# Amos-Chen98/neo-planner

Measured on AMD Instinct MI355X. Metric: trajectories/sec (batched replan), higher is better.
Workload: dtype f32x; 1 GPU; cfg2: 40 x 4096 trajectories x 20 waypoints per step per GPU, 1 x 300^3 f32 ESDF per GPU (trilinear, pillars + 80 canopy boxes), each optimised to L-BFGS-B termination; batch_per_launch=4096, pieces=21, dims=3, esdf_voxels=27000000, layout=brick, parallelism=scene-sharded x1, launches_in_flight_per_gpu=4

## Files before the change

### neo-planner_amd/csrc/neo_group_kernel.hpp

```cpp
#pragma once
#include "neo_device.hpp"
#include "neo_lbfgs_sm.hpp"

namespace neo {

template <int D, int W, int NS, typename Real, class MapT, class LookupT, int SU, typename Num = double>
struct GroupBackend {
  using Hist = Num;
  struct Vec {
    Num v[NS];
  };
  Traj<D, D, Num> t;
  const DevParams &prm;
  const MapT &map;
  double *xs;
  double *sc;
  LineSearch *lsp;
  double *cst;
  Hist *hist;
  int m;

  __device__ GroupBackend(const DevParams &p, const MapT &mp) : prm(p), map(mp) {}

  __device__ __forceinline__ double dot(const Vec &a, const Vec &b) const {
    Num s = Num(0);
#pragma unroll
    for (int k = 0; k < NS; ++k) s += a.v[k] * b.v[k];
    return GroupLanes<W>::sum(s);
  }
  __device__ __forceinline__ double amax(const Vec &a) const {
    Num s = Num(0);
#pragma unroll
    for (int k = 0; k < NS; ++k) s = fmax(s, fabs(a.v[k]));
    return GroupLanes<W>::max_nonneg(s);
  }
  __device__ __forceinline__ void copy(Vec &d, const Vec &s) const {
#pragma unroll
    for (int k = 0; k < NS; ++k) d.v[k] = s.v[k];
  }
  __device__ __forceinline__ void neg(Vec &d, const Vec &s) const {
#pragma unroll
    for (int k = 0; k < NS; ++k) d.v[k] = -s.v[k];
  }
  __device__ __forceinline__ void axpy(double a, const Vec &x, Vec &y) const {
#pragma unroll
    for (int k = 0; k < NS; ++k) y.v[k] += (Num)a * x.v[k];
  }
  __device__ __forceinline__ void lincomb(Vec &o, const Vec &a, double s, const Vec &b) const {
#pragma unroll
    for (int k = 0; k < NS; ++k) o.v[k] = a.v[k] + (Num)s * b.v[k];
  }
  __device__ __forceinline__ void scale(Vec &v, double s) const {
#pragma unroll
    for (int k = 0; k < NS; ++k) v.v[k] *= (Num)s;
  }
  __device__ __forceinline__ void hist_put(int slot, const Vec &s, const Vec &y) {
    const int gl = GroupLanes<W>::lane();
#pragma unroll
    for (int k = 0; k < NS; ++k)
      if (k * W + gl < t.n) {
        hist[slot * t.n + k * W + gl] = s.v[k];
        hist[(m + slot) * t.n + k * W + gl] = y.v[k];
      }
    lds_wave_sync();
  }
  __device__ __forceinline__ void hist_get(int row, Vec &v) const {
    const int gl = GroupLanes<W>::lane();
#pragma unroll
    for (int k = 0; k < NS; ++k) v.v[k] = (k * W + gl < t.n) ? hist[row * t.n + k * W + gl] : Num(0);
  }
  __device__ __forceinline__ void hist_get_s(int slot, Vec &v) const { hist_get(slot, v); }
  __device__ __forceinline__ void hist_get_y(int slot, Vec &v) const { hist_get(m + slot, v); }
  __device__ __forceinline__ void hist_get_sy(int slot, Vec &s, Vec &y) const {
    hist_get(slot, s);
    hist_get(m + slot, y);
  }
  __device__ __forceinline__ void sput(int i, double v) {
    sc[i] = v;
    lds_wave_sync();
  }
  __device__ __forceinline__ double sget(int i) const { return sc[i]; }
  __device__ __forceinline__ double sdiff(int i, double b) const { return sget(i) - b; }
  __device__ __forceinline__ double rho_dot(int slot, const Vec &a, const Vec &b) const { return sget(slot) * dot(a, b); }
  __device__ __forceinline__ double uni(double v) const { return v; }
  __device__ __forceinline__ LineSearch &ls() { return *lsp; }
  __device__ __forceinline__ double *cost_store() { return cst; }
  __device__ __forceinline__ void note_eval(int, int, double, double, const Vec &, const Vec &) {}

  __device__ __forceinline__ int eval(const Vec &x, double &f, Vec &g, double (&costs)[4], int &nsamp) {
    const int lane = GroupLanes<W>::lane();
    const int M = t.M;
    Num *xn = reinterpret_cast<Num *>(xs);
    lds_wave_sync();
#pragma unroll
    for (int k = 0; k < NS; ++k)
      if (k * W + lane < t.n) xn[k * W + lane] = x.v[k];
    lds_wave_sync();
    const bool act = lane < M;
    t.tau = act ? xn[t.nq + lane] : Num(0);
#pragma unroll
    for (int d = 0; d < D; ++d) {
      t.P0[d] = (lane == 0 || !act) ? bstate<D, GroupLanes<W>, false>(t, 0, d) : xn[d * (M - 1) + (lane > 0 ? lane - 1 : 0)];
      t.P1[d] = (lane >= M - 1) ? bstate<D, GroupLanes<W>, true>(t, 0, d) : xn[d * (M - 1) + lane];
    }
    double energy = 0.0, tsum = 0.0;
    const int st = minco_forward<D, GroupLanes<W>, Num>(t, prm, energy, tsum);
    nsamp = GroupLanes<W>::sum(act ? t.ns : 0);
    Num gC[6][D], gT = Num(0);
    double cf, ck;
    {
      Real cr[6][D], gCr[6][D], gTr;
#pragma unroll
      for (int k = 0; k < 6; ++k)
#pragma unroll
        for (int d = 0; d < D; ++d) cr[k][d] = (Real)t.c[k][d];
      LookupT lk(map);
      const SampleLanes sl = group_sample_lanes<GroupLanes<W>>(M, t.ns);
      minco_sample<Real, D, LookupT, SU, false, GroupLanes<W>>(M, sl, t.ns, cr, prm, lk, gCr, gTr, cf, ck);
#pragma unroll
      for (int k = 0; k < 6; ++k)
#pragma unroll
        for (int d = 0; d < D; ++d) gC[k][d] = (Num)gCr[k][d];
      gT = (Num)gTr;
    }
    costs[0] = energy;
    costs[1] = tsum;
    costs[2] = cf;
    costs[3] = ck;
    f = costs[0] * prm.w[0] + costs[1] * prm.w[1] + costs[2] * prm.w[2] + costs[3] * prm.w[3];
    Num gq[D], gtau;
    const int bst = minco_backward<D, GroupLanes<W>, Num>(t, prm, gC, gT, gq, gtau);
    lds_wave_sync();
    if (lane >= 1 && lane < M) {
#pragma unroll
      for (int d = 0; d < D; ++d) xn[d * (M - 1) + lane - 1] = gq[d];
    }
    if (lane < M) xn[t.nq + lane] = gtau;
    lds_wave_sync();
#pragma unroll
    for (int k = 0; k < NS; ++k) g.v[k] = (k * W + lane < t.n) ? xn[k * W + lane] : Num(0);
    if (st != 0) {
      f = 0.0;
#pragma unroll
      for (int k = 0; k < 4; ++k) costs[k] = 0.0;
      return st;
    }
    return bst;
  }
};

#ifndef NEO_GRP_OCC
#define NEO_GRP_OCC 1
#endif
#ifndef NEO_GRP_OCC_F32
#define NEO_GRP_OCC_F32 2
#endif
#ifndef NEO_GRP_U
#define NEO_GRP_U 2
#endif
template <int D, typename Real, class MapT, class LookupT, int W, int NS, typename Num = double>
__global__ __launch_bounds__(kWave, (sizeof(Num) == 4 ? NEO_GRP_OCC_F32 : NEO_GRP_OCC)) void optimize_group_kernel(int B, int M, DevParams prm, const MapT *maps,
                                                                   const double *x0, double *x,
                                                                   const double *__restrict__ head,
                                                                   const double *__restrict__ tail,
                                                                   double *__restrict__ costs4,
                                                                   double *__restrict__ costs4_last,
                                                                   int *__restrict__ nit, int *__restrict__ nfev,
                                                                   int *__restrict__ status,
                                                                   long long *__restrict__ nsamples,
                                                                   const int *__restrict__ order,
                                                                   int *__restrict__ ticket) {
  constexpr int G = kWave / W;
  __shared__ double xs[G][W * NS];
  __shared__ double sc[G][2 * NEO_LBFGS_M];
  __shared__ LineSearch lsm[G];
  __shared__ double cst[G][12];
  __shared__ Num bnd[G][6 * D];
  extern __shared__ double dyn_lds[];
  using BE = GroupBackend<D, W, NS, Real, MapT, LookupT, NEO_GRP_U, Num>;
  const MapT map = maps[0];
  BE be(prm, map);
  be.t = Traj<D, D, Num>{};
  const int gl = GroupLanes<W>::lane();
  const int g = lane_id() / W;
  const int nq = D * (M - 1), n = nq + M;
  be.xs = xs[g];
  be.sc = sc[g];
  be.lsp = &lsm[g];
  be.cst = cst[g];
  be.m = NEO_LBFGS_M;
  be.hist = reinterpret_cast<typename BE::Hist *>(dyn_lds) + (size_t)g * 2 * NEO_LBFGS_M * n;
  be.t.M = M;
  be.t.nq = nq;
  be.t.n = n;
  be.t.L = GroupLanes<W>::lanes_per_piece(M);
  be.t.bnd = bnd[g];

  LbfgsOpts o{prm.ftol, prm.gtol, prm.maxls, prm.maxiter, prm.maxfun, NEO_LBFGS_M};
  LbfgsMachine<BE> mach(be, o);
  int b = 0;
  bool busy = false;
  long long samples = 0;

  auto take = [&]() {
    int tk = 0;
    if (gl == 0) tk = atomicAdd(ticket, 1);
    tk = __shfl(tk, GroupLanes<W>::base(), kWave);
    busy = tk < B;
    b = busy ? (order ? order[tk] : tk) : 0;
    be.t.head = head + (size_t)b * 3 * D;
    be.t.tail = tail + (size_t)b * 3 * D;
    lds_wave_sync();
    for (int e = gl; e < 6 * D; e += W)
      bnd[g][e] = (Num)(e < 3 * D ? be.t.head[e] : be.t.tail[e - 3 * D]);
    lds_wave_sync();
#pragma unroll
    for (int k = 0; k < NS; ++k) mach.x.v[k] = (k * W + gl < n) ? x0[(size_t)b * n + k * W + gl] : 0.0;
    mach.begin();
    samples = 0;
  };
  auto put = [&]() {
#pragma unroll
    for (int k = 0; k < NS; ++k)
      if (k * W + gl < n) x[(size_t)b * n + k * W + gl] = mach.x.v[k];
    if (gl == 0) {
      LbfgsResult res;
      mach.result(res);
      int st = res.status;
      if (res.costs_last[3] * prm.w[3] > prm.coll_tol) st |= NEO_TRAJ_FLAG_COLLISION;
#pragma unroll
      for (int k = 0; k < 4; ++k) {
        costs4[(size_t)b * 4 + k] = res.costs[k];
        if (costs4_last) costs4_last[(size_t)b * 4 + k] = res.costs_last[k];
      }
      nit[b] = res.nit;
      nfev[b] = res.nfev;
      status[b] = st;
      if (nsamples) nsamples[b] = samples;
    }
  };

  take();
  while (__any(busy)) {
    double fnew, c4[4];
    typename BE::Vec gnew;
    int ns;
    const int est = be.eval(mach.x, fnew, gnew, c4, ns);
    if (busy) {
      mach.f = fnew;
      mach.g = gnew;
#pragma unroll
      for (int k = 0; k < 4; ++k) be.cst[k] = c4[k];
      samples += ns;
      mach.advance(est);
      if (!mach.need_eval()) {
        put();
        take();
      }
    }
  }
}

}
```

### neo-planner_amd/csrc/neo_kernels.hpp

```cpp
#pragma once
#include <type_traits>
#include <hip/hip_runtime.h>
#include <hip/hip_fp16.h>

#include "../../include/neo_planner.h"
#ifndef NEO_FUSED_U
#define NEO_FUSED_U (sizeof(Real) == 4 ? 4 : 2)
#endif
#ifndef NEO_W2_U
#define NEO_W2_U 1
#endif
#ifndef NEO_W2_OCC
#define NEO_W2_OCC 2
#endif
#ifndef NEO_X_OCC
#define NEO_X_OCC 3
#endif
#ifndef NEO_SM_MAX_SLOTS
#define NEO_SM_MAX_SLOTS 2
#endif
#ifndef NEO_W2_MAX_SLOTS
#define NEO_W2_MAX_SLOTS 4
#endif
#include "neo_device.hpp"
#include "neo_lbfgs.hpp"
#include "neo_lbfgs_sm.hpp"

namespace neo {

template <typename Num, int NS>
using opt_scalar_t = std::conditional_t<sizeof(Num) == 4 && (NS <= NEO_SM_MAX_SLOTS), float, double>;

template <int D, int NS, typename Real>
__host__ __device__ constexpr int stage_doubles() {
  constexpr int fold = sizeof(Real) == 4 ? kWave * 8 * D * (int)sizeof(Real) : 0;
  return (NS * kWave * 8 > fold ? NS * kWave * 8 : fold) / 8;
}

constexpr int kSlCacheInts = kWave / 4 + kWave + 4;

template <typename Real, int NS, int WAVES>
__host__ __device__ constexpr bool pairs_in_f32() {
  return sizeof(Real) == 4 && WAVES == 2 && NS > 2;
}
template <int D, int NS, typename Real, class MapT, class LookupT, int SU = NEO_FUSED_U, class LG = WaveLanes,
          bool PAIRS32 = false, typename Num = double, class Plan = PlanDynamic>
struct DevBackend {
  static constexpr int DL = LG::dl(D);
  static constexpr int kSlotsN = NS;
  static constexpr bool kPcr = sizeof(Num) == 4 && LG::W == kWave;
  static constexpr bool kAhead = !Plan::dynamic && Plan::gather_ahead && LookupT::gather_ahead && SU == 1 && sizeof(Real) == 4;
  struct Vec {
    Num v[NS];
  };
  Traj<D, DL, Num> t;
  const DevParams &prm;
  const MapT &map;
  double *xs;
  static constexpr int kStage = stage_doubles<D, NS, Real>();
  int *sl_cache = nullptr;
  bool fold_rows = true;
  bool fold_acc = false;
  using Scalar = opt_scalar_t<Num, NS>;
  LineSearchT<Scalar> *lsp;
  double *cst;
  using Hist = std::conditional_t<PAIRS32, float, double>;
  Hist *hist;
  int npad, m;
  double *coeff_out;
  long long samples = 0;
  int last_ns = 0;
  double *trace = nullptr;
  double *trace_xg = nullptr;
  int trace_cap = 0;

  __device__ DevBackend(const DevParams &p, const MapT &mp) : prm(p), map(mp) {}

  __device__ __forceinline__ double dot(const Vec &a, const Vec &b) const {
    Num s = Num(0);
#pragma unroll
    for (int k = 0; k < NS; ++k) s += a.v[k] * b.v[k];
    return uni((double)wave_sum(s));
  }
  __device__ __forceinline__ double uni(double v) const { return uniform(v); }
  __device__ __forceinline__ float uni(float v) const { return uniform(v); }
  __device__ __forceinline__ double amax(const Vec &a) const {
    Num s = Num(0);
#pragma unroll
    for (int k = 0; k < NS; ++k) s = fmax(s, fabs(a.v[k]));
    return wave_max_nonneg(s);
  }
  __device__ __forceinline__ void copy(Vec &d, const Vec &s) const {
#pragma unroll
    for (int k = 0; k < NS; ++k) d.v[k] = s.v[k];
  }
  __device__ __forceinline__ void neg(Vec &d, const Vec &s) const {
#pragma unroll
    for (int k = 0; k < NS; ++k) d.v[k] = -s.v[k];
  }
  __device__ __forceinline__ void axpy(double a, const Vec &x, Vec &y) const {
#pragma unroll
    for (int k = 0; k < NS; ++k) y.v[k] += (Num)a * x.v[k];
  }
  __device__ __forceinline__ void lincomb(Vec &o, const Vec &a, double s, const Vec &b) const {
#pragma unroll
    for (int k = 0; k < NS; ++k) o.v[k] = a.v[k] + (Num)s * b.v[k];
  }
  __device__ __forceinline__ void scale(Vec &v, double s) const {
#pragma unroll
    for (int k = 0; k < NS; ++k) v.v[k] *= (Num)s;
  }
  static constexpr int kFull = NS == 3 ? 2 : NS / 2;
  __device__ __forceinline__ bool in_range(int k, int lane) const { return k < kFull || k * kWave + lane < t.n; }
  __device__ __forceinline__ void hist_put(int slot, const Vec &s, const Vec &y) {
    const int lane = lane_id();
#pragma unroll
    for (int k = 0; k < NS; ++k)
      if (in_range(k, lane)) {
        hist[slot * t.n + k * kWave + lane] = (Hist)s.v[k];
        hist[(m + slot) * t.n + k * kWave + lane] = (Hist)y.v[k];
      }
    lds_wave_sync();
  }
  __device__ __forceinline__ void hist_get(int row, Vec &v) const {
    const int lane = lane_id();
#pragma unroll
    for (int k = 0; k < NS; ++k) v.v[k] = in_range(k, lane) ? (Num)hist[row * t.n + k * kWave + lane] : Num(0);
  }
  __device__ __forceinline__ void hist_get_s(int slot, Vec &v) const { hist_get(slot, v); }
  __device__ __forceinline__ void hist_get_y(int slot, Vec &v) const { hist_get(m + slot, v); }
  __device__ __forceinline__ void hist_get_sy(int slot, Vec &s, Vec &y) const {
    const int lane = lane_id();
    const Hist *ps = hist + slot * t.n + lane, *py = hist + (m + slot) * t.n + lane;
#pragma unroll
    for (int k = 0; k < NS; ++k) {
      s.v[k] = Num(0);
      y.v[k] = Num(0);
      if (in_range(k, lane)) {
        s.v[k] = (Num)ps[k * kWave];
        y.v[k] = (Num)py[k * kWave];
      }
    }
  }
  Num sreg = Num(0);
  __device__ __forceinline__ void sput(int i, double v) { sreg = (lane_id() == i) ? (Num)v : sreg; }
  __device__ __forceinline__ double sget(int i) const { return (double)rdlane(sreg, i); }
  __device__ __forceinline__ double sdiff(int i, double b) const { return (double)(rdlane(sreg, i) - (Num)b); }
  __device__ __forceinline__ double rho_dot(int slot, const Vec &a, const Vec &b) const {
    Num s = Num(0);
#pragma unroll
    for (int k = 0; k < NS; ++k) s += a.v[k] * b.v[k];
    return (double)(rdlane(sreg, slot) * wave_sum(s));
  }
  static constexpr bool kOwnDirection = sizeof(Num) == 4;
  __device__ __forceinline__ void dot3(const Vec &a0, const Vec &b0, const Vec &a1, const Vec &b1, const Vec &a2, const Vec &b2,
                                       Num &t0, Num &t1, Num &t2) const {
    Num p0 = Num(0), p1 = Num(0), p2 = Num(0);
#pragma unroll
    for (int k = 0; k < NS; ++k) {
      p0 += a0.v[k] * b0.v[k];
      p1 += a1.v[k] * b1.v[k];
      p2 += a2.v[k] * b2.v[k];
    }
    Num unused;
    wave_sum4((float)p0, (float)p1, (float)p2, 0.0f, t0, t1, t2, unused);
  }
  __device__ __forceinline__ void direction(const Vec &g, Vec &d, int col, int head, int mm, Num theta) {
    if (col == 0) {
      neg(d, g);
      return;
    }
    if constexpr (!Plan::dynamic && Plan::hist_ahead) {
      if (col == NEO_LBFGS_M) {
        direction_full(g, d, head, mm, theta);
        return;
      }
    }
    auto slot_of = [&](int k) { return head + k < mm ? head + k : head + k - mm; };
    copy(d, g);
    Vec sA, yA, sB, yB;
    int k = col - 1;
    for (; k >= 1; k -= 2) {
      const int A = slot_of(k), B = slot_of(k - 1);
      hist_get_sy(A, sA, yA);
      hist_get_sy(B, sB, yB);
      Num t0, t1, t2;
      dot3(sA, d, sB, d, sB, yA, t0, t1, t2);
      const Num aA = rdlane(sreg, A) * t0;
      const Num aB = rdlane(sreg, B) * (t1 - aA * t2);
      sput(mm + A, (double)aA);
      sput(mm + B, (double)aB);
#pragma unroll
      for (int q = 0; q < NS; ++q) d.v[q] = (d.v[q] - aA * yA.v[q]) - aB * yB.v[q];
    }
    if (k == 0) {
      const int A = slot_of(0);
      hist_get_sy(A, sA, yA);
      const Num aA = (Num)rho_dot(A, sA, d);
      sput(mm + A, (double)aA);
      axpy(-(double)aA, yA, d);
    }
    scale(d, (double)(Num(1) / theta));
    k = 0;
    for (; k + 1 < col; k += 2) {
      const int A = slot_of(k), B = slot_of(k + 1);
      hist_get_sy(A, sA, yA);
      hist_get_sy(B, sB, yB);
      Num t0, t1, t2;
      dot3(yA, d, yB, d, yB, sA, t0, t1, t2);
      const Num cA = rdlane(sreg, mm + A) - rdlane(sreg, A) * t0;
      const Num cB = rdlane(sreg, mm + B) - rdlane(sreg, B) * (t1 + cA * t2);
#pragma unroll
      for (int q = 0; q < NS; ++q) d.v[q] = (d.v[q] + cA * sA.v[q]) + cB * sB.v[q];
    }
    if (k < col) {
      const int A = slot_of(k);
      hist_get_sy(A, sA, yA);
      const double b = rho_dot(A, yA, d);
      axpy(sdiff(mm + A, b), sA, d);
    }
    scale(d, -1.0);
  }
  template <int COL>
  struct DirFull {
    DevBackend &be;
    Vec &d;
    const Num inv_theta;
    int off[NS];
    Vec s[COL], y[COL];
    Num alpha[COL];
    __device__ __forceinline__ void settle(Vec &sv, Vec &yv) const {
#pragma unroll
      for (int k = kFull; k < NS; ++k)
        if (lane_ge(be.t.n - k * kWave)) {
          sv.v[k] = Num(0);
          yv.v[k] = Num(0);
        }
    }
    template <int K>
    __device__ __forceinline__ void read(int slot) {
      const Hist *ps = be.hist + slot * be.t.n, *py = be.hist + (be.m + slot) * be.t.n;
#pragma unroll
      for (int k = 0; k < NS; ++k) {
        s[K].v[k] = (Num)ps[off[k]];
        y[K].v[k] = (Num)py[off[k]];
      }
    }
    template <int KA, int KB>
    __device__ __forceinline__ void pair1(int A, int B) {
      settle(s[KA], y[KA]);
      settle(s[KB], y[KB]);
      Num t0, t1, t2;
      be.dot3(s[KA], d, s[KB], d, s[KB], y[KA], t0, t1, t2);
      const Num aA = rdlane(be.sreg, A) * t0;
      const Num aB = rdlane(be.sreg, B) * (t1 - aA * t2);
      alpha[KA] = aA;
      alpha[KB] = aB;
#pragma unroll
      for (int q = 0; q < NS; ++q) d.v[q] = (d.v[q] - aA * y[KA].v[q]) - aB * y[KB].v[q];
    }
    template <int KA, int KB>
    __device__ __forceinline__ void pair2(int A, int B) {
      Num t0, t1, t2;
      be.dot3(y[KA], d, y[KB], d, y[KB], s[KA], t0, t1, t2);
      const Num cA = alpha[KA] - rdlane(be.sreg, A) * t0;
      const Num cB = alpha[KB] - rdlane(be.sreg, B) * (t1 + cA * t2);
#pragma unroll
      for (int q = 0; q < NS; ++q) d.v[q] = (d.v[q] + cA * s[KA].v[q]) + cB * s[KB].v[q];
    }
    template <int K>
    __device__ __forceinline__ void single1(int A) {
      settle(s[K], y[K]);
      const Num aA = (Num)be.rho_dot(A, s[K], d);
      alpha[K] = aA;
      be.axpy(-(double)aA, y[K], d);
    }
    template <int K>
    __device__ __forceinline__ void single2(int A) {
      const double b = be.rho_dot(A, y[K], d);
      be.axpy((double)(alpha[K] - (Num)b), s[K], d);
    }
    __device__ __forceinline__ void seam() { be.scale(d, (double)inv_theta); }
  };
  __device__ __forceinline__ void direction_full(const Vec &g, Vec &d, int head, int mm, Num theta) {
    copy(d, g);
    DirFull<NEO_LBFGS_M> w{*this, d, Num(1) / theta};
    const int lane = lane_id();
#pragma unroll
    for (int k = 0; k < NS; ++k) w.off[k] = in_range(k, lane) ? k * kWave + lane : 0;
    hist_walk_full<NEO_LBFGS_M>(head, mm, w);
    scale(d, -1.0);
  }

  __device__ __forceinline__ LineSearchT<Scalar> &ls() { return *lsp; }
  __device__ __forceinline__ double *cost_store() { return cst; }

  __device__ __forceinline__ void note_eval(int nfev, int iter, double stp, double f, const Vec &x, const Vec &g) {
    if constexpr (!Plan::dynamic && !Plan::trace) return;
    if (nfev > trace_cap) return;
    if (trace != nullptr && lane_id() == 0) {
      double *r = trace + (size_t)(nfev - 1) * 4;
      r[0] = f;
      r[1] = stp;
      r[2] = (double)last_ns;
      r[3] = (double)iter;
    }
    if (trace_xg != nullptr) {
      const int lane = lane_id();
      double *r = trace_xg + (size_t)(nfev - 1) * 2 * t.n;
#pragma unroll
      for (int k = 0; k < NS; ++k)
        if (k * kWave + lane < t.n) {
          r[k * kWave + lane] = (double)x.v[k];
          r[t.n + k * kWave + lane] = (double)g.v[k];
        }
    }
  }

  __device__ __forceinline__ void scatter_x(const Vec &x) {
    const int lane = opaque(lane_id());
    lds_wave_sync();
    Num *xn = reinterpret_cast<Num *>(xs);
#pragma unroll
    for (int k = 0; k < NS; ++k)
      if (in_range(k, lane)) xn[k * kWave + lane] = x.v[k];
    lds_wave_sync();
    const int M = t.M;
    const int p = opaque(LG::piece());
    const bool act = p < M;
    t.tau = act ? xn[t.nq + p] : Num(0);
#pragma unroll
    for (int d = 0; d < DL; ++d) {
      const int dg = LG::dim0() + d;
      t.P0[d] = (p == 0 || !act) ? bstate<D, LG, false>(t, 0, d) : xn[dg * (M - 1) + (p > 0 ? p - 1 : 0)];
      t.P1[d] = (p >= M - 1) ? bstate<D, LG, true>(t, 0, d) : xn[dg * (M - 1) + p];
    }
  }

  __device__ __forceinline__ int eval(const Vec &x, double &f, Vec &g, double *costs) {
    const int lane = lane_id();
    const int p = LG::piece();
    NEO_MARK("eval_begin");
    const int M_all = t.M;
    t.M = opaque_uniform(M_all);
    scatter_x(x);
    NEO_MARK("scatter_done");
    Num *xn = reinterpret_cast<Num *>(xs);
    double energy, tsum;
    const int st = minco_forward<D, LG, Num, kPcr, Plan>(t, prm, energy, tsum);
    NEO_MARK("forward_done");
    if (st != 0) {
      f = 0.0;
#pragma unroll
      for (int k = 0; k < 4; ++k) costs[k] = 0.0;
      return st;
    }
    if (plan_pick<Plan, Plan::coeff_out>(coeff_out != nullptr) && p < t.M) {
#pragma unroll
      for (int k = 0; k < 6; ++k)
#pragma unroll
        for (int d = 0; d < DL; ++d) coeff_out[(size_t)(6 * p + k) * D + LG::dim0() + d] = (double)t.c[k][d];
    }
    Num gC[6][DL], gT = Num(0);
    double cf, ck;
    {
      Real cr[6][DL], gCr[6][DL], gTr;
#pragma unroll
      for (int k = 0; k < 6; ++k)
#pragma unroll
        for (int d = 0; d < DL; ++d) cr[k][d] = (Real)t.c[k][d];
      LookupT lk(map);
      int ns_by_piece = t.ns;
      if constexpr (LG::S > 1) ns_by_piece = __shfl(t.ns, min(LG::S * lane, kWave - 1), kWave);
      NEO_MARK("assign_begin");
      t.M = opaque_uniform(M_all);
      SampleLanes sl;
      bool cached = false;
      const int ns_key = lane < t.M ? ns_by_piece : 0;
      const bool have_cache = plan_pick<Plan, Plan::sl_cache>(sl_cache != nullptr);
      if (have_cache) cached = __ballot(ns_key == (int)reinterpret_cast<const unsigned char *>(sl_cache)[lane]) == ~0ull;
      if (cached) {
        const unsigned pk = (unsigned)sl_cache[kWave / 4 + lane];
        sl.piece = pk & 63;
        sl.r = (pk >> 6) & 63;
        sl.L = (pk >> 12) & 127;
        sl.act = ((pk >> 19) & 1) != 0;
        sl.first = (pk >> 20) & 63;
        sl.Lp = pk >> 26;
        sl.rounds = __builtin_amdgcn_readfirstlane(sl_cache[kWave / 4 + kWave]);
        sl.lmax = __builtin_amdgcn_readfirstlane(sl_cache[kWave / 4 + kWave + 1]);
        sl.total = __builtin_amdgcn_readfirstlane(sl_cache[kWave / 4 + kWave + 2]);
      } else {
        sl = balanced_sample_lanes<kAhead>(t.M, ns_by_piece, reinterpret_cast<int *>(xs));
        if (have_cache) {
          const bool fits = sl.lmax < 64 && ns_key < 255;
          reinterpret_cast<unsigned char *>(sl_cache)[lane] = (unsigned char)(__ballot(!fits) == 0 ? ns_key : 255);
          sl_cache[kWave / 4 + lane] = (int)((unsigned)sl.piece | ((unsigned)sl.r << 6) | ((unsigned)sl.L << 12) |
                                             ((sl.act ? 1u : 0u) << 19) | ((unsigned)sl.first << 20) | ((unsigned)sl.Lp << 26));
          if (lane == 0) {
            sl_cache[kWave / 4 + kWave] = sl.rounds;
            sl_cache[kWave / 4 + kWave + 1] = sl.lmax;
            sl_cache[kWave / 4 + kWave + 2] = sl.total;
          }
          lds_wave_sync();
        }
      }
      last_ns = sl.total;
      samples += (long long)last_ns;
      NEO_MARK("assign_done");
      minco_sample<Real, D, LookupT, SU, false, LG, Plan>(
          t.M, sl, t.ns, cr, prm, lk, gCr, gTr, cf, ck,
          plan_pick<Plan, Plan::fold_rows>(fold_rows) ? reinterpret_cast<Real *>(xs) : nullptr, fold_acc);
#pragma unroll
      for (int k = 0; k < 6; ++k)
#pragma unroll
        for (int d = 0; d < DL; ++d) gC[k][d] = (Num)gCr[k][d];
      gT = (Num)gTr;
    }
    costs[0] = uniform(energy);
    costs[1] = uniform(tsum);
    costs[2] = uniform(cf);
    costs[3] = uniform(ck);
    f = uniform(costs[0] * prm.w[0] + costs[1] * prm.w[1] + costs[2] * prm.w[2] + costs[3] * prm.w[3]);
    Num gq[DL], gtau;
    NEO_MARK("sample_done");
    t.M = opaque_uniform(M_all);
    if constexpr (kAhead && sizeof(Num) == 4) {
      const Num i1 = opaque(t.i1);
      t.i2 = i1 * i1;
      t.i3 = t.i2 * i1;
      t.i4 = t.i2 * t.i2;
    }
    const int bst = minco_backward<D, LG, Num, kPcr, Plan>(t, prm, gC, gT, gq, gtau);
    NEO_MARK("backward_done");
    if (bst != 0) return bst;
    lds_wave_sync();
    const int pg = opaque(p), lg = opaque(lane);
    if (pg >= 1 && pg < t.M) {
#pragma unroll
      for (int d = 0; d < DL; ++d) xn[(LG::dim0() + d) * (t.M - 1) + pg - 1] = gq[d];
    }
    if (pg < t.M && LG::dim0() == opaque_uniform(0)) xn[t.nq + pg] = gtau;
    lds_wave_sync();
#pragma unroll
    for (int k = 0; k < NS; ++k) g.v[k] = in_range(k, lg) ? xn[k * kWave + lg] : Num(0);
    NEO_MARK("gather_done");
    return 0;
  }
};

__host__ __device__ inline size_t opt_state_doubles(int n, int m) { return 64 + 5 * (size_t)n + kWave + 2 * (size_t)m * (size_t)n; }

template <class BE, class Mach>
__device__ __forceinline__ void save_run(BE &be, const Mach &mc, double *st) {
  const int lane = lane_id(), n = be.t.n;
  lds_wave_sync();
  if (lane == 0) {
    const int iv[9] = {mc.phase, mc.status, mc.nfev, mc.nit, mc.iter, mc.col, mc.head, mc.task, mc.ifun};
#pragma unroll
    for (int k = 0; k < 9; ++k) st[k] = (double)iv[k];
    const double dv[7] = {(double)mc.f, (double)mc.fold, (double)mc.stp, (double)mc.gd, (double)mc.gdold, (double)mc.theta,
                          (double)mc.stp_evaluated};
#pragma unroll
    for (int k = 0; k < 7; ++k) st[9 + k] = dv[k];
    st[16] = (double)be.samples;
    st[17] = (double)be.last_ns;
    const auto &L = *be.lsp;
    const double lv[20] = {(double)L.ftol, (double)L.gtol, (double)L.xtol, (double)L.stpmin, (double)L.stpmax, (double)L.brackt,
                           (double)L.stage, (double)L.ginit, (double)L.gtest, (double)L.gx, (double)L.gy, (double)L.finit,
                           (double)L.fx, (double)L.fy, (double)L.stx, (double)L.sty, (double)L.stmin, (double)L.stmax,
                           (double)L.width, (double)L.width1};
#pragma unroll
    for (int k = 0; k < 20; ++k) st[20 + k] = lv[k];
#pragma unroll
    for (int k = 0; k < 12; ++k) st[40 + k] = be.cst[k];
  }
  double *v = st + 64;
#pragma unroll
  for (int k = 0; k < BE::kSlotsN; ++k)
    if (k * kWave + lane < n) {
      const int e = k * kWave + lane;
      v[e] = (double)mc.x.v[k];
      v[n + e] = (double)mc.g.v[k];
      v[2 * n + e] = (double)mc.t.v[k];
      v[3 * n + e] = (double)mc.r.v[k];
      v[4 * n + e] = (double)mc.d.v[k];
    }
  v[5 * n + lane] = (double)be.sreg;
  double *h = v + 5 * n + kWave;
  for (int i = lane; i < 2 * be.m * n; i += kWave) h[i] = (double)be.hist[i];
}

template <class BE, class Mach>
__device__ __forceinline__ void load_run(BE &be, Mach &mc, const double *st) {
  using Num = decltype(be.sreg);
  const int lane = lane_id(), n = be.t.n;
  auto iu = [&](int k) { return (int)uniform(st[k]); };
  mc.phase = iu(0); mc.status = iu(1); mc.nfev = iu(2); mc.nit = iu(3); mc.iter = iu(4);
  mc.col = iu(5); mc.head = iu(6); mc.task = iu(7); mc.ifun = iu(8);
  using S = typename Mach::S;
  mc.f = (S)uniform(st[9]); mc.fold = (S)uniform(st[10]); mc.stp = (S)uniform(st[11]); mc.gd = (S)uniform(st[12]);
  mc.gdold = (S)uniform(st[13]); mc.theta = (S)uniform(st[14]); mc.stp_evaluated = (S)uniform(st[15]);
  be.samples = (long long)uniform(st[16]);
  be.last_ns = iu(17);
  if (lane == 0) {
    auto &L = *be.lsp;
    L.ftol = (S)st[20]; L.gtol = (S)st[21]; L.xtol = (S)st[22]; L.stpmin = (S)st[23]; L.stpmax = (S)st[24];
    L.brackt = (int)st[25]; L.stage = (int)st[26];
    L.ginit = (S)st[27]; L.gtest = (S)st[28]; L.gx = (S)st[29]; L.gy = (S)st[30]; L.finit = (S)st[31]; L.fx = (S)st[32];
    L.fy = (S)st[33]; L.stx = (S)st[34]; L.sty = (S)st[35]; L.stmin = (S)st[36]; L.stmax = (S)st[37]; L.width = (S)st[38];
    L.width1 = (S)st[39];
#pragma unroll
    for (int k = 0; k < 12; ++k) be.cst[k] = st[40 + k];
  }
  const double *v = st + 64;
#pragma unroll
  for (int k = 0; k < BE::kSlotsN; ++k) {
    const int e = k * kWave + lane;
    const bool in = e < n;
    mc.x.v[k] = in ? (Num)v[e] : Num(0);
    mc.g.v[k] = in ? (Num)v[n + e] : Num(0);
    mc.t.v[k] = in ? (Num)v[2 * n + e] : Num(0);
    mc.r.v[k] = in ? (Num)v[3 * n + e] : Num(0);
    mc.d.v[k] = in ? (Num)v[4 * n + e] : Num(0);
  }
  be.sreg = (Num)v[5 * n + lane];
  const double *h = v + 5 * n + kWave;
  for (int i = lane; i < 2 * be.m * n; i += kWave) be.hist[i] = (typename BE::Hist)h[i];
  lds_wave_sync();
}

template <class LG = WaveLanes, int D, int DL, typename Num>
__device__ __forceinline__ void load_boundary(Traj<D, DL, Num> &t, const double *head, const double *tail, int M,
                                              Num *bnd_lds = nullptr) {
  t.M = M;
  t.nq = D * (M - 1);
  t.n = t.nq + M;
  t.L = sample_lanes_per_piece(M);
  t.head = head;
  t.tail = tail;
  stage_boundary<D, LG>(t, bnd_lds);
}

struct MapTable {
  const void *maps;
};

template <int D, int NS, typename Real, class MapT, class LookupT, class LG = WaveLanes, typename Num = double>
__global__ __launch_bounds__(kWave) void eval_kernel(int B, int M, DevParams prm, MapT map,
                                                      const double *__restrict__ x,
                                                      const double *__restrict__ head,
                                                      const double *__restrict__ tail,
                                                      double *__restrict__ cost, double *__restrict__ costs4,
                                                      double *__restrict__ grad, double *__restrict__ coeffs,
                                                      int *__restrict__ status) {
  __shared__ __attribute__((aligned(16))) double xs[stage_doubles<D, NS, Real>()];
  __shared__ LineSearchT<opt_scalar_t<Num, NS>> lsm;
  __shared__ double cst[12];
  __shared__ Num bnd[6 * D];
  constexpr bool kKeep = sizeof(Num) == 4 && LG::S > 1;
  __shared__ __attribute__((aligned(16))) Num mult_s[kKeep ? (5 * 8 + 4) * (kWave / LG::S + 1) : 4];
  const int b = blockIdx.x;
  if (b >= B) return;
  using BE = DevBackend<D, NS, Real, MapT, LookupT, NEO_FUSED_U, LG, false, Num>;
  BE be(prm, map);
  if constexpr (kKeep) be.t.pcr_mult = mult_s;
  be.xs = xs;
  if constexpr (sizeof(Num) == 4 && LG::W == kWave)
    if (pcr_xch_elems(M, LG::dl(D)) * (int)sizeof(Num) <= stage_doubles<D, NS, Real>() * 8) be.t.pcr_xch = reinterpret_cast<Num *>(xs);
  be.lsp = &lsm;
  be.cst = cst;
  be.hist = nullptr;
  be.m = NEO_LBFGS_M;
  load_boundary<LG>(be.t, head + (size_t)b * 3 * D, tail + (size_t)b * 3 * D, M, bnd);
  const int n = be.t.n;
  be.npad = NS * kWave;
  be.coeff_out = coeffs ? coeffs + (size_t)b * 6 * M * D : nullptr;
  const int lane = lane_id();
  typename BE::Vec xv, gv;
#pragma unroll
  for (int k = 0; k < NS; ++k) xv.v[k] = (k * kWave + lane < n) ? x[(size_t)b * n + k * kWave + lane] : 0.0;
  double f;
  double *costs = cst;
  const int st = be.eval(xv, f, gv, costs);
#pragma unroll
  for (int k = 0; k < NS; ++k)
    if (k * kWave + lane < n) grad[(size_t)b * n + k * kWave + lane] = gv.v[k];
  if (lane == 0) {
    cost[b] = f;
#pragma unroll
    for (int k = 0; k < 4; ++k) costs4[(size_t)b * 4 + k] = costs[k];
    if (status) status[b] = st;
// ... 264 lines not shown
```

### neo-planner_amd/csrc/neo_launch_opt.hpp

```cpp
#pragma once
#include "neo_host.hpp"
#include "neo_kernels.hpp"

namespace neo {

struct OptLds {
  int stage, pcr_off;
  size_t dyn;
};

template <int D, int NS, typename Real, int WAVES, class LG, typename Num>
OptLds opt_lds_plan(int M, int flags, int stash = 0) {
  const size_t pair_elems = (size_t)2 * NEO_LBFGS_M * (D * (M - 1) + M);
  const size_t cache = sizeof(Num) == 4 ? kSlCacheInts * sizeof(int) : 0;
  const size_t statics = 400;
  const size_t lds_share8 = (size_t)160 * 1024 / 8 / 1280 * 1280 - statics - cache,
               lds_share12 = (size_t)160 * 1024 / (4 * NEO_X_OCC) / 1280 * 1280 - statics - cache;
  const size_t pairs = pair_elems * ((pairs_in_f32<Real, NS, WAVES>() || sizeof(Num) == 4) ? sizeof(float) : sizeof(double));
  const int full = stage_doubles<D, NS, Real>(), small = NS * kWave;
  const size_t lds_share = (sizeof(Num) == 4 && NS <= 2) ? lds_share12 : lds_share8;
  OptLds l{pairs + (size_t)full * 8 <= lds_share ? full : small, 0, 0};
  l.dyn = pairs + (size_t)l.stage * 8;
  if (sizeof(Num) == 4 && LG::S > 1 && !(flags & 4096)) {
    const int acc = std::max(std::max(std::max(small, (M * fold_acc_stride(D) * 4 + 7) / 8), (pcr_xch_elems(M, 1) * 4 + 7) / 8),
                             (stash + 7) / 8);
    const size_t off = ((size_t)acc * 8 + pairs + 15) / 16 * 2;
    const size_t need = off * 8 + (size_t)pcr_mult_elems(M) * sizeof(float);
    if (need <= lds_share) {
      l.stage = acc;
      l.pcr_off = (int)off;
      l.dyn = need;
    }
  }
  return l;
}

template <int D, int NS, typename Real, class MapT, class LookupT, int WAVES, class LG, typename Num, bool BUDGET>
int launch_opt_kernel(neo_ctx *c, const OptArgs &a) {
  const int n_launch = a.subset ? a.n_subset : a.B;
  const int *launch_order = a.subset ? a.subset : (c->order_B == a.B ? c->dispatch_order : nullptr);
  constexpr int stash = opt_gather_ahead<D, NS, Real, MapT, LookupT, WAVES, LG, Num, BUDGET>() ? velocity_stash_bytes(D) : 0;
  const OptLds l = opt_lds_plan<D, NS, Real, WAVES, LG, Num>(a.M, c->params.flags, stash);
  using Plan = opt_plan_t<NS, LG, Num, BUDGET>;
  bool fixed = !Plan::dynamic;
  if constexpr (!Plan::dynamic)
    fixed = l.pcr_off != 0 && pcr_xch_elems(a.M, LG::dl(D)) * (int)sizeof(Num) <= l.stage * 8 && stash <= l.stage * 8 &&
            !c->trace && !c->trace_xg && !(c->params.flags & 4096);
  auto kernel = optimize_kernel<D, NS, Real, MapT, LookupT, WAVES, LG, Num, BUDGET>;
  if constexpr (!Plan::dynamic)
    if (!fixed) kernel = optimize_dyn_kernel<D, NS, Real, MapT, LookupT, WAVES, LG, Num, BUDGET>;
  ++c->opt_plan_launches[fixed ? 0 : 1];
  hipLaunchKernelGGL(kernel, dim3(n_launch), dim3(kWave), l.dyn,
                     c->stream, n_launch, a.M, c->dev, static_cast<const MapT *>(a.table), a.slots, a.nmaps,
                     a.x0 ? a.x0 : a.x, a.x, a.head, a.tail, a.costs4, a.costs4_last, a.nit, a.nfev, a.status,
                     c->sample_counter, launch_order, c->trace, c->trace_xg, c->trace_cap, l.stage, l.pcr_off,
                     BUDGET ? a.state : reinterpret_cast<double *>(c->progress) ,
                     a.state_doubles, a.budget, a.resume, a.traj_total);
  return NEO_OK;
}

template <int D, typename Real, class MapT, class LookupT, int WAVES = 1, typename Num = double, bool BUDGET = false>
int launch_opt(neo_ctx *c, const OptArgs &a) {
  constexpr int max_ns = BUDGET ? 2 : (WAVES == 1 || NEO_W2_MAX_SLOTS >= 4) ? 4 : 2;
  if (const int ns = slots_for(a.M, D); ns > max_ns) {
    if (BUDGET) return fail(c, NEO_ERR_INVALID, "budgeted launches: n <= 128 variables");
    if (ns == 3) return fail(c, NEO_ERR_INVALID, "n > 128 variables: this build has no two-waves kernel for three FLAT slots");
    return fail(c, NEO_ERR_INVALID, "n > 128 variables: this build has no two-waves kernel for four FLAT slots "
                                    "(NEO_W2_MAX_SLOTS < 4)");
  }
  return visit_slots<D, max_ns>(a.M, c->params.flags, [&](auto ns, auto lg) {
    return launch_opt_kernel<D, decltype(ns)::value, Real, MapT, LookupT, WAVES, type_of<decltype(lg)>, Num, BUDGET>(c, a);
  });
}

}
```

### neo-planner_amd/csrc/neo_lbfgs_dir.hpp

```cpp
#pragma once
#include <type_traits>

namespace neo {

template <class Backend, class = void>
struct has_own_direction { static constexpr bool value = false; };
template <class Backend>
struct has_own_direction<Backend, std::enable_if_t<Backend::kOwnDirection>> { static constexpr bool value = true; };

NEO_HD int hist_slot(int head, int k, int m) { return head + k < m ? head + k : head + k - m; }
template <int K, class V>
NEO_HD void hist_full_read1(int head, int m, V &v) {
  if constexpr (K >= 0) v.template read<K>(hist_slot(head, K, m));
  if constexpr (K >= 1) v.template read<K - 1>(hist_slot(head, K - 1, m));
}
template <int K, class V>
NEO_HD void hist_full_loop1(int head, int m, V &v) {
  if constexpr (K >= 0) hist_full_read1<K - 2>(head, m, v);
  if constexpr (K >= 1) {
    v.template pair1<K, K - 1>(hist_slot(head, K, m), hist_slot(head, K - 1, m));
    hist_full_loop1<K - 2>(head, m, v);
  } else if constexpr (K == 0) {
    v.template single1<0>(hist_slot(head, 0, m));
  }
}
template <int COL, int K, class V>
NEO_HD void hist_full_loop2(int head, int m, V &v) {
  if constexpr (K + 1 < COL) {
    v.template pair2<K, K + 1>(hist_slot(head, K, m), hist_slot(head, K + 1, m));
    hist_full_loop2<COL, K + 2>(head, m, v);
  } else if constexpr (K < COL) {
    v.template single2<K>(hist_slot(head, K, m));
  }
}
template <int COL, class V>
NEO_HD void hist_walk_full(int head, int m, V &v) {
  static_assert(COL >= 1, "at least one pair");
  hist_full_read1<COL - 1>(head, m, v);
  hist_full_loop1<COL - 1>(head, m, v);
  v.seam();
  hist_full_loop2<COL, 0>(head, m, v);
}

template <class Backend>
NEO_HD void lbfgs_direction(Backend &be, const typename Backend::Vec &g, typename Backend::Vec &d,
                            typename Backend::Vec &tmp, typename Backend::Vec &tmp2, int col, int head, int m,
                            double theta) {
  if constexpr (has_own_direction<Backend>::value) {
    be.direction(g, d, col, head, m, theta);
    return;
  }
  if (col == 0) {
    be.neg(d, g);
    return;
  }
  be.copy(d, g);
  for (int k = col - 1; k >= 0; --k) {
    const int slot = head + k < m ? head + k : head + k - m;
    be.hist_get_sy(slot, tmp, tmp2);
    const double a = be.rho_dot(slot, tmp, d);
    be.sput(m + slot, a);
    be.axpy(-a, tmp2, d);
  }
  be.scale(d, 1.0 / theta);
  for (int k = 0; k < col; ++k) {
    const int slot = head + k < m ? head + k : head + k - m;
    be.hist_get_sy(slot, tmp2, tmp);
    const double b = be.rho_dot(slot, tmp, d);
    be.axpy(be.sdiff(m + slot, b), tmp2, d);
  }
  be.scale(d, -1.0);
}

}
```

### neo-planner_amd/csrc/neo_wave.hpp

```cpp
#pragma once
#include <type_traits>
#include <hip/hip_runtime.h>

namespace neo {

constexpr int kWave = 64;

__device__ __forceinline__ int lane_id() { return (int)__lane_id(); }

__device__ __forceinline__ void lds_wave_sync() {
#ifdef NEO_STRONG_SYNC
  __syncthreads();
#else
  __builtin_amdgcn_fence(__ATOMIC_ACQ_REL, "wavefront");
  __builtin_amdgcn_wave_barrier();
#endif
}

__device__ __forceinline__ double precise_rcp(double d) {
  double r = __builtin_amdgcn_rcp(d);
  r = fma(fma(-d, r, 1.0), r, r);
  r = fma(fma(-d, r, 1.0), r, r);
  return r;
}
__device__ __forceinline__ float precise_rcp(float d) { return __builtin_amdgcn_rcpf(d); }
#ifdef NEO_MARKS
#define NEO_MARK(name) asm volatile("; NEOMARK " name)
#else
#define NEO_MARK(name)
#endif
__device__ __forceinline__ int opaque(int v) {
  asm volatile("" : "+v"(v));
  return v;
}
__device__ __forceinline__ float opaque(float v) {
  asm volatile("" : "+v"(v));
  return v;
}
__device__ __forceinline__ int opaque_uniform(int v) {
  asm volatile("" : "+s"(v));
  return v;
}
__device__ __forceinline__ bool lane_lt(int bound) { return (int)__lane_id() < opaque_uniform(bound); }
__device__ __forceinline__ bool lane_ge(int bound) { return (int)__lane_id() >= opaque_uniform(bound); }
__device__ __forceinline__ bool lane_eq(int which) { return (int)__lane_id() == opaque_uniform(which); }

template <class T>
constexpr bool is_lane_type = std::is_same<T, int>::value || std::is_same<T, float>::value || std::is_same<T, double>::value;
#define NEO_MAP_WORDS(T, v, WORD_OP)                                                              \
  static_assert(is_lane_type<T>, "cross-lane primitives take exactly int, float or double");      \
  if constexpr (std::is_same<T, int>::value) {                                                    \
    const int w = v;                                                                              \
    return WORD_OP;                                                                               \
  } else if constexpr (std::is_same<T, float>::value) {                                           \
    const int w = __float_as_int(v);                                                              \
    return __int_as_float(WORD_OP);                                                               \
  } else {                                                                                        \
    int w = __double2loint(v);                                                                    \
    const int lo = WORD_OP;                                                                       \
    w = __double2hiint(v);                                                                        \
    const int hi = WORD_OP;                                                                       \
    return __hiloint2double(hi, lo);                                                              \
  }

template <class T>
__device__ __forceinline__ T rdlane(T v, int src ) {
  NEO_MAP_WORDS(T, v, __builtin_amdgcn_readlane(w, src))
}
template <class T>
__device__ __forceinline__ T uniform(T v) {
  NEO_MAP_WORDS(T, v, __builtin_amdgcn_readfirstlane(w))
}

template <int CTRL, int ROW_MASK = 0xf>
__device__ __forceinline__ int dpp_i(int v) {
  return __builtin_amdgcn_update_dpp(0, v, CTRL, ROW_MASK, 0xf, ROW_MASK == 0xf);
}
template <int CTRL, int ROW_MASK = 0xf, class T>
__device__ __forceinline__ T dpp(T v) {
  NEO_MAP_WORDS(T, v, (dpp_i<CTRL, ROW_MASK>(w)))
}
template <int CTRL, int ROW_MASK>
__device__ __forceinline__ int dpp_any_i(int v) {
  return __builtin_amdgcn_mov_dpp(v, CTRL, ROW_MASK, 0xf, false);
}
template <int CTRL, int ROW_MASK, class T>
__device__ __forceinline__ T dpp_any(T v) {
  NEO_MAP_WORDS(T, v, (dpp_any_i<CTRL, ROW_MASK>(w)))
}
template <int CTRL, int ROW_MASK = 0xf, class T>
__device__ __forceinline__ T dpp_keep(T v) {
  NEO_MAP_WORDS(T, v, __builtin_amdgcn_update_dpp(w, w, CTRL, ROW_MASK, 0xf, false))
}
struct FillZero {
  template <int CTRL, int ROW_MASK, class T>
  static __device__ __forceinline__ T move(T v) { return dpp<CTRL, ROW_MASK>(v); }
};
struct FillAny {
  template <int CTRL, int ROW_MASK, class T>
  static __device__ __forceinline__ T move(T v) { return dpp_any<CTRL, ROW_MASK>(v); }
};

template <class Fill = FillZero, class T, class Op>
__device__ __forceinline__ T row_scan(T v, Op op) {
  v = op(v, Fill::template move<0x111, 0xf>(v));
  v = op(v, Fill::template move<0x112, 0xf>(v));
  v = op(v, Fill::template move<0x114, 0xf>(v));
  v = op(v, Fill::template move<0x118, 0xf>(v));
  return v;
}
template <class Fill = FillZero, class BcastFill = Fill, class T, class Op>
__device__ __forceinline__ T wave_scan(T v, Op op) {
  v = row_scan<Fill>(v, op);
  v = op(v, BcastFill::template move<0x142, 0xa>(v));
  v = op(v, BcastFill::template move<0x143, 0xc>(v));
  return v;
}
template <class T, class Op>
__device__ __forceinline__ T wave_reduce(T v, Op op) {
  return rdlane(wave_scan<FillZero, FillAny>(v, op), kWave - 1);
}
struct OpAdd {
  template <class T>
  __device__ __forceinline__ T operator()(T a, T b) const { return a + b; }
};
struct OpMax {
  __device__ __forceinline__ int operator()(int a, int b) const { return max(a, b); }
  __device__ __forceinline__ float operator()(float a, float b) const { return fmaxf(a, b); }
  __device__ __forceinline__ double operator()(double a, double b) const { return fmax(a, b); }
};
template <class T>
__device__ __forceinline__ T wave_sum(T v) { return wave_reduce(v, OpAdd()); }
template <class T>
__device__ __forceinline__ T wave_max_nonneg(T v) { return wave_reduce(v, OpMax()); }
__device__ __forceinline__ int wave_sum(int v) {
  v += dpp<0x111>(v);
  v += dpp<0x112>(v);
  v += dpp<0x114>(v);
  v += dpp<0x118>(v);
  v += dpp_any<0x142, 0xa>(v);
  v += dpp_any<0x143, 0xc>(v);
  return rdlane(v, kWave - 1);
}
__device__ __forceinline__ int wave_scan_add(int v) {
  v += dpp<0x111>(v);
  v += dpp<0x112>(v);
  v += dpp<0x114>(v);
  v += dpp<0x118>(v);
  v += dpp<0x142, 0xa>(v);
  v += dpp<0x143, 0xc>(v);
  return v;
}
__device__ __forceinline__ int wave_scan_max_nonneg(int v) { return wave_scan(v, OpMax()); }

template <class T, class F>
__device__ __forceinline__ void swap_words(T &x, T &y, F f) {
  static_assert(std::is_same<T, float>::value || std::is_same<T, double>::value, "float or double");
  if constexpr (std::is_same<T, float>::value) {
    const auto r = f(__float_as_uint(x), __float_as_uint(y));
    x = __uint_as_float(r[0]);
    y = __uint_as_float(r[1]);
  } else {
    const auto lo = f((unsigned)__double2loint(x), (unsigned)__double2loint(y));
    const auto hi = f((unsigned)__double2hiint(x), (unsigned)__double2hiint(y));
    x = __hiloint2double((int)hi[0], (int)lo[0]);
    y = __hiloint2double((int)hi[1], (int)lo[1]);
  }
}
template <class T>
__device__ __forceinline__ void swap_half_waves(T &x, T &y) {
  swap_words(x, y, [](unsigned a, unsigned b) { return __builtin_amdgcn_permlane32_swap(a, b, false, false); });
}
template <class T>
__device__ __forceinline__ void swap_odd_even_rows(T &x, T &y) {
  swap_words(x, y, [](unsigned a, unsigned b) { return __builtin_amdgcn_permlane16_swap(a, b, false, false); });
}
template <class T>
__device__ __forceinline__ void wave_sum4(T a, T b, T c, T d, T &ta, T &tb, T &tc, T &td) {
  swap_half_waves(a, c);
  T x = a + c;
  swap_half_waves(b, d);
  T y = b + d;
  swap_odd_even_rows(x, y);
  T z = x + y;
  z = row_scan(z, OpAdd());
  ta = rdlane(z, 15);
  tb = rdlane(z, 31);
  tc = rdlane(z, 47);
  td = rdlane(z, 63);
}

template <class T>
__device__ __forceinline__ T from_prev(T v, T fill) {
  const T o = dpp<0x138>(v);
  return lane_eq(0) ? fill : o;
}
template <class T>
__device__ __forceinline__ T from_next(T v, T fill) {
  const T o = dpp<0x130>(v);
  return lane_eq(kWave - 1) ? fill : o;
}

#undef NEO_MAP_WORDS

}
```

Baseline: 1.679 million traj/s.

## Interleave L-BFGS s/y history into paired records for single vector LDS loads

When history is stored in 32-bit floats, the L-BFGS s and y vectors are now stored interleaved as float2 records instead of in two separate row blocks. Each history read then pulls s and y with one 64-bit LDS access. The full-history direction walk drops its per-lane clamped offset array and reads unmasked records. The fixed-plan check is extended to reserve LDS for the resulting over-read past n. This is meant to halve LDS load instructions and cut address arithmetic in the two-loop recursion, at the risk of over-reading into neighbouring LDS and pushing more launches onto the dynamic kernel.

```diff
diff --git a/neo-planner_amd/csrc/neo_group_kernel.hpp b/neo-planner_amd/csrc/neo_group_kernel.hpp
--- a/neo-planner_amd/csrc/neo_group_kernel.hpp
+++ b/neo-planner_amd/csrc/neo_group_kernel.hpp
@@ -19,6 +19,9 @@
   double *cst;
   Hist *hist;
   int m;
+  static constexpr bool kRecords = sizeof(Hist) == 4;
+  typedef Hist HistPair __attribute__((ext_vector_type(2)));
+  __device__ __forceinline__ HistPair *hist_rec(int slot) const { return reinterpret_cast<HistPair *>(hist) + hist_record(slot, 0, t.n); }
 
   __device__ GroupBackend(const DevParams &p, const MapT &mp) : prm(p), map(mp) {}
 
@@ -59,21 +62,40 @@
 #pragma unroll
     for (int k = 0; k < NS; ++k)
       if (k * W + gl < t.n) {
-        hist[slot * t.n + k * W + gl] = s.v[k];
-        hist[(m + slot) * t.n + k * W + gl] = y.v[k];
-      }
-    lds_wave_sync();
-  }
-  __device__ __forceinline__ void hist_get(int row, Vec &v) const {
+        if constexpr (kRecords) {
+          hist_rec(slot)[k * W + gl] = HistPair{opaque(s.v[k]), opaque(y.v[k])};
+        } else {
+          hist[hist_index_rows(slot, k * W + gl, t.n, m, 0)] = s.v[k];
+          hist[hist_index_rows(slot, k * W + gl, t.n, m, 1)] = y.v[k];
+        }
+      }
+    lds_wave_sync();
+  }
+  template <int WHICH>
+  __device__ __forceinline__ void hist_get(int slot, Vec &v) const {
     const int gl = GroupLanes<W>::lane();
 #pragma unroll
-    for (int k = 0; k < NS; ++k) v.v[k] = (k * W + gl < t.n) ? hist[row * t.n + k * W + gl] : Num(0);
-  }
-  __device__ __forceinline__ void hist_get_s(int slot, Vec &v) const { hist_get(slot, v); }
-  __device__ __forceinline__ void hist_get_y(int slot, Vec &v) const { hist_get(m + slot, v); }
+    for (int k = 0; k < NS; ++k) {
+      const int e = k * W + gl;
+      v.v[k] = (e < t.n) ? hist[kRecords ? hist_index(slot, e, t.n, WHICH) : hist_index_rows(slot, e, t.n, m, WHICH)] : Num(0);
+    }
+  }
+  __device__ __forceinline__ void hist_get_s(int slot, Vec &v) const { hist_get<0>(slot, v); }
+  __device__ __forceinline__ void hist_get_y(int slot, Vec &v) const { hist_get<1>(slot, v); }
   __device__ __forceinline__ void hist_get_sy(int slot, Vec &s, Vec &y) const {
-    hist_get(slot, s);
-    hist_get(m + slot, y);
+    if constexpr (kRecords) {
+      const int gl = GroupLanes<W>::lane();
+#pragma unroll
+      for (int k = 0; k < NS; ++k) {
+        const bool in = k * W + gl < t.n;
+        const HistPair r = hist_rec(slot)[in ? k * W + gl : 0];
+        s.v[k] = in ? r.x : Num(0);
+        y.v[k] = in ? r.y : Num(0);
+      }
+    } else {
+      hist_get<0>(slot, s);
+      hist_get<1>(slot, y);
+    }
   }
   __device__ __forceinline__ void sput(int i, double v) {
     sc[i] = v;
diff --git a/neo-planner_amd/csrc/neo_kernels.hpp b/neo-planner_amd/csrc/neo_kernels.hpp
--- a/neo-planner_amd/csrc/neo_kernels.hpp
+++ b/neo-planner_amd/csrc/neo_kernels.hpp
@@ -112,33 +112,71 @@
   }
   static constexpr int kFull = NS == 3 ? 2 : NS / 2;
   __device__ __forceinline__ bool in_range(int k, int lane) const { return k < kFull || k * kWave + lane < t.n; }
+  static constexpr bool kRecords = sizeof(Hist) == 4;
+  typedef Hist HistPair __attribute__((ext_vector_type(2)));
+  __device__ __forceinline__ HistPair *hist_rec(int slot, int e) const {
+    return reinterpret_cast<HistPair *>(hist) + hist_record(slot, e, t.n);
+  }
   __device__ __forceinline__ void hist_put(int slot, const Vec &s, const Vec &y) {
     const int lane = lane_id();
-#pragma unroll
-    for (int k = 0; k < NS; ++k)
-      if (in_range(k, lane)) {
-        hist[slot * t.n + k * kWave + lane] = (Hist)s.v[k];
-        hist[(m + slot) * t.n + k * kWave + lane] = (Hist)y.v[k];
-      }
+    if constexpr (kRecords) {
+      HistPair *p = hist_rec(slot, lane);
+#pragma unroll
+      for (int k = 0; k < NS; ++k)
+        if (in_range(k, lane)) p[k * kWave] = HistPair{(Hist)opaque(s.v[k]), (Hist)opaque(y.v[k])};
+    } else {
+#pragma unroll
+      for (int k = 0; k < NS; ++k)
+        if (in_range(k, lane)) {
+          hist[hist_index_rows(slot, k * kWave + lane, t.n, m, 0)] = (Hist)s.v[k];
+          hist[hist_index_rows(slot, k * kWave + lane, t.n, m, 1)] = (Hist)y.v[k];
+        }
+    }
     lds_wave_sync();
   }
-  __device__ __forceinline__ void hist_get(int row, Vec &v) const {
+  template <int WHICH>
+  __device__ __forceinline__ void hist_get(int slot, Vec &v) const {
     const int lane = lane_id();
 #pragma unroll
-    for (int k = 0; k < NS; ++k) v.v[k] = in_range(k, lane) ? (Num)hist[row * t.n + k * kWave + lane] : Num(0);
-  }
-  __device__ __forceinline__ void hist_get_s(int slot, Vec &v) const { hist_get(slot, v); }
-  __device__ __forceinline__ void hist_get_y(int slot, Vec &v) const { hist_get(m + slot, v); }
+    for (int k = 0; k < NS; ++k) {
+      const int e = k * kWave + lane;
+      v.v[k] = in_range(k, lane) ? (Num)hist[kRecords ? hist_index(slot, e, t.n, WHICH) : hist_index_rows(slot, e, t.n, m, WHICH)] : Num(0);
+    }
+  }
+  __device__ __forceinline__ void hist_get_s(int slot, Vec &v) const { hist_get<0>(slot, v); }
+  __device__ __forceinline__ void hist_get_y(int slot, Vec &v) const { hist_get<1>(slot, v); }
+  static constexpr bool kMaskedRead = sizeof(Num) == 8 && NS == 3;
   __device__ __forceinline__ void hist_get_sy(int slot, Vec &s, Vec &y) const {
     const int lane = lane_id();
-    const Hist *ps = hist + slot * t.n + lane, *py = hist + (m + slot) * t.n + lane;
-#pragma unroll
-    for (int k = 0; k < NS; ++k) {
-      s.v[k] = Num(0);
-      y.v[k] = Num(0);
-      if (in_range(k, lane)) {
-        s.v[k] = (Num)ps[k * kWave];
-        y.v[k] = (Num)py[k * kWave];
+    if constexpr (kRecords) {
+      const HistPair *p = hist_rec(slot, 0);
+#pragma unroll
+      for (int k = 0; k < NS; ++k) {
+        const bool in = in_range(k, lane);
+        if constexpr (kMaskedRead) {
+          s.v[k] = Num(0);
+          y.v[k] = Num(0);
+          if (in) {
+            const HistPair r = p[k * kWave + lane];
+            s.v[k] = (Num)r.x;
+            y.v[k] = (Num)r.y;
+          }
+        } else {
+          const HistPair r = p[in ? k * kWave + lane : 0];
+          s.v[k] = in ? (Num)r.x : Num(0);
+          y.v[k] = in ? (Num)r.y : Num(0);
+        }
+      }
+    } else {
+      const Hist *ps = hist + hist_index_rows(slot, lane, t.n, m, 0), *py = hist + hist_index_rows(slot, lane, t.n, m, 1);
+#pragma unroll
+      for (int k = 0; k < NS; ++k) {
+        s.v[k] = Num(0);
+        y.v[k] = Num(0);
+        if (in_range(k, lane)) {
+          s.v[k] = (Num)ps[k * kWave];
+          y.v[k] = (Num)py[k * kWave];
+        }
       }
     }
   }
@@ -226,7 +264,6 @@
     DevBackend &be;
     Vec &d;
     const Num inv_theta;
-    int off[NS];
     Vec s[COL], y[COL];
     Num alpha[COL];
     __device__ __forceinline__ void settle(Vec &sv, Vec &yv) const {
@@ -239,11 +276,12 @@
     }
     template <int K>
     __device__ __forceinline__ void read(int slot) {
-      const Hist *ps = be.hist + slot * be.t.n, *py = be.hist + (be.m + slot) * be.t.n;
+      const HistPair *p = be.hist_rec(slot, lane_id());
 #pragma unroll
       for (int k = 0; k < NS; ++k) {
-        s[K].v[k] = (Num)ps[off[k]];
-        y[K].v[k] = (Num)py[off[k]];
+        const HistPair r = p[k * kWave];
+        s[K].v[k] = (Num)r.x;
+        y[K].v[k] = (Num)r.y;
       }
     }
     template <int KA, int KB>
@@ -285,9 +323,6 @@
   __device__ __forceinline__ void direction_full(const Vec &g, Vec &d, int head, int mm, Num theta) {
     copy(d, g);
     DirFull<NEO_LBFGS_M> w{*this, d, Num(1) / theta};
-    const int lane = lane_id();
-#pragma unroll
-    for (int k = 0; k < NS; ++k) w.off[k] = in_range(k, lane) ? k * kWave + lane : 0;
     hist_walk_full<NEO_LBFGS_M>(head, mm, w);
     scale(d, -1.0);
   }
diff --git a/neo-planner_amd/csrc/neo_launch_opt.hpp b/neo-planner_amd/csrc/neo_launch_opt.hpp
--- a/neo-planner_amd/csrc/neo_launch_opt.hpp
+++ b/neo-planner_amd/csrc/neo_launch_opt.hpp
@@ -35,6 +35,14 @@
   return l;
 }
 
+template <int D, int NS, class LG, typename Num>
+bool opt_plan_fixed(const OptLds &l, int M, int stash, bool plain) {
+  const int n = D * (M - 1) + M;
+  const size_t pairs_end = (size_t)l.stage * 8 + (size_t)2 * NEO_LBFGS_M * n * sizeof(Num);
+  return l.pcr_off != 0 && pcr_xch_elems(M, LG::dl(D)) * (int)sizeof(Num) <= l.stage * 8 && stash <= l.stage * 8 &&
+         pairs_end + (size_t)hist_over_read_elems(n, NS * kWave) * sizeof(Num) <= l.dyn && plain;
+}
+
 template <int D, int NS, typename Real, class MapT, class LookupT, int WAVES, class LG, typename Num, bool BUDGET>
 int launch_opt_kernel(neo_ctx *c, const OptArgs &a) {
   const int n_launch = a.subset ? a.n_subset : a.B;
@@ -44,8 +52,7 @@
   using Plan = opt_plan_t<NS, LG, Num, BUDGET>;
   bool fixed = !Plan::dynamic;
   if constexpr (!Plan::dynamic)
-    fixed = l.pcr_off != 0 && pcr_xch_elems(a.M, LG::dl(D)) * (int)sizeof(Num) <= l.stage * 8 && stash <= l.stage * 8 &&
-            !c->trace && !c->trace_xg && !(c->params.flags & 4096);
+    fixed = opt_plan_fixed<D, NS, LG, Num>(l, a.M, stash, !c->trace && !c->trace_xg && !(c->params.flags & 4096));
   auto kernel = optimize_kernel<D, NS, Real, MapT, LookupT, WAVES, LG, Num, BUDGET>;
   if constexpr (!Plan::dynamic)
     if (!fixed) kernel = optimize_dyn_kernel<D, NS, Real, MapT, LookupT, WAVES, LG, Num, BUDGET>;
diff --git a/neo-planner_amd/csrc/neo_lbfgs_dir.hpp b/neo-planner_amd/csrc/neo_lbfgs_dir.hpp
--- a/neo-planner_amd/csrc/neo_lbfgs_dir.hpp
+++ b/neo-planner_amd/csrc/neo_lbfgs_dir.hpp
@@ -9,6 +9,11 @@
 struct has_own_direction<Backend, std::enable_if_t<Backend::kOwnDirection>> { static constexpr bool value = true; };
 
 NEO_HD int hist_slot(int head, int k, int m) { return head + k < m ? head + k : head + k - m; }
+
+NEO_HD int hist_record(int slot, int e, int n) { return slot * n + e; }
+NEO_HD int hist_index(int slot, int e, int n, int which) { return hist_record(slot, e, n) * 2 + which; }
+NEO_HD int hist_index_rows(int slot, int e, int n, int m, int which) { return (which * m + slot) * n + e; }
+NEO_HD int hist_over_read_elems(int n, int lanes) { return (lanes - n) * 2; }
 template <int K, class V>
 NEO_HD void hist_full_read1(int head, int m, V &v) {
   if constexpr (K >= 0) v.template read<K>(hist_slot(head, K, m));
diff --git a/neo-planner_amd/csrc/neo_wave.hpp b/neo-planner_amd/csrc/neo_wave.hpp
--- a/neo-planner_amd/csrc/neo_wave.hpp
+++ b/neo-planner_amd/csrc/neo_wave.hpp
@@ -34,6 +34,10 @@
   return v;
 }
 __device__ __forceinline__ float opaque(float v) {
+  asm volatile("" : "+v"(v));
+  return v;
+}
+__device__ __forceinline__ double opaque(double v) {
   asm volatile("" : "+v"(v));
   return v;
 }
```

Result: faster. 1.713 million traj/s, median of 6 (+2.0%).
